# mathaiml5/NBody-simulation-parallel

Hardware: AMD Instinct MI355X
Metric: body-pair interactions/sec at N=2^20 (all-pairs force + kick/drift step) (higher is better)
Workload: dtype f32

## Files before the change

### nbody-simulation-parallel_amd/csrc/force_sym_kernel.hip

```cpp
#include "nbx_internal.h"
#include "sym_plan.h"

namespace nbx {
namespace {

typedef float f2 __attribute__((ext_vector_type(2)));

__device__ __forceinline__ float ror1(float v) {
    const int i = __builtin_bit_cast(int, v);
    return __builtin_bit_cast(float, __builtin_amdgcn_update_dpp(i, i, 0x13C, 0xF, 0xF, false));
}
__device__ __forceinline__ void ror1(f2& v) { v.x = ror1(v.x); v.y = ror1(v.y); }

enum { kRotDpp = 0, kRotLds = 1 };
template <int D> struct RotBuf { static constexpr unsigned kEntries = (D == 3) ? 128u : 72u; };

template <int D, int PAIRS>
__device__ __forceinline__ void sym_step(const f2 vxy, const f2 vzm, const f2 (&ix)[PAIRS], const f2 (&iy)[PAIRS],
                                         const f2 (&iz)[PAIRS], const f2 (&hm)[PAIRS], f2 (&ax)[PAIRS], f2 (&ay)[PAIRS],
                                         f2 (&az)[PAIRS], f2& vax, f2& vay, f2& vaz, const f2 bias) {
    f2 dx[PAIRS], dy[PAIRS], dz[PAIRS], r2[PAIRS], w[PAIRS], wh[PAIRS];
#pragma unroll
    for (int q = 0; q < PAIRS; ++q) dx[q] = __builtin_shufflevector(vxy, vxy, 0, 0) - ix[q];
#pragma unroll
    for (int q = 0; q < PAIRS; ++q) dy[q] = __builtin_shufflevector(vxy, vxy, 1, 1) - iy[q];
#pragma unroll
    for (int q = 0; q < PAIRS; ++q) dz[q] = (D == 3) ? __builtin_shufflevector(vzm, vzm, 0, 0) - iz[q] : f2{0.f, 0.f};
#pragma unroll
    for (int q = 0; q < PAIRS; ++q) r2[q] = __builtin_elementwise_fma(dx[q], dx[q], bias);
#pragma unroll
    for (int q = 0; q < PAIRS; ++q) r2[q] = __builtin_elementwise_fma(dy[q], dy[q], r2[q]);
    if (D == 3) {
#pragma unroll
        for (int q = 0; q < PAIRS; ++q) r2[q] = __builtin_elementwise_fma(dz[q], dz[q], r2[q]);
    }
#pragma unroll
    for (int q = 0; q < PAIRS; ++q) { w[q].x = __builtin_amdgcn_rcpf(r2[q].x); w[q].y = __builtin_amdgcn_rcpf(r2[q].y); }
#pragma unroll
    for (int q = 0; q < PAIRS; ++q) r2[q] = w[q] * w[q];
#pragma unroll
    for (int q = 0; q < PAIRS; ++q) w[q] = __builtin_shufflevector(vzm, vzm, 1, 1) * r2[q];
#pragma unroll
    for (int q = 0; q < PAIRS; ++q) wh[q] = hm[q] * r2[q];
#pragma unroll
    for (int q = 0; q < PAIRS; ++q) ax[q] = __builtin_elementwise_fma(w[q], dx[q], ax[q]);
#pragma unroll
    for (int q = 0; q < PAIRS; ++q) ay[q] = __builtin_elementwise_fma(w[q], dy[q], ay[q]);
    if (D == 3) {
#pragma unroll
        for (int q = 0; q < PAIRS; ++q) az[q] = __builtin_elementwise_fma(w[q], dz[q], az[q]);
    }
#pragma unroll
    for (int q = 0; q < PAIRS; ++q) {
        vax = __builtin_elementwise_fma(wh[q], dx[q], vax);
        vay = __builtin_elementwise_fma(wh[q], dy[q], vay);
        if (D == 3) vaz = __builtin_elementwise_fma(wh[q], dz[q], vaz);
    }
}

template <int D>
__device__ __forceinline__ void load_visitor(const float* __restrict__ tp, const float* __restrict__ mp, unsigned pad,
                                             unsigned v, f2& vxy, f2& vzm) {
    vxy = f2{tp[v], tp[(size_t)pad + v]};
    vzm = f2{(D == 3) ? tp[2 * (size_t)pad + v] : 0.0f, mp[v]};
}

__device__ __forceinline__ void store_hi_lo(float* __restrict__ hi_plane, float* __restrict__ lo_plane, size_t idx, double v) {
    const float hi = (float)v;
    hi_plane[idx] = hi;
    lo_plane[idx] = (float)(v - (double)hi);
}

template <int D, int QS, int ROT>
__global__ __launch_bounds__(256, 2) void accel_sym3l_kernel(KArgs a) {
    constexpr int PAIRS = 4;
    constexpr unsigned kSumBytes = (unsigned)PAIRS * D * 256u * sizeof(double2);
    constexpr unsigned kVisBytes = 4u * kSymChunkGroups * kSymGroup * sizeof(float4);
    constexpr unsigned kRotEntries = RotBuf<D>::kEntries;
    constexpr unsigned kRotBytes = (ROT == kRotLds) ? 4u * kRotEntries * sizeof(float4) : 0u;
    __shared__ __attribute__((aligned(16))) char smem[kSumBytes + kVisBytes + kRotBytes];
    double2* __restrict__ sums = reinterpret_cast<double2*>(smem);
    float4* __restrict__ vbuf = reinterpret_cast<float4*>(smem + kSumBytes);

    SymPlan P;
    if (!sym_make_plan(a.pad, &P) || P.B != gridDim.x || P.S != gridDim.y) return;
    const unsigned A = blockIdx.x, s = blockIdx.y;
    const unsigned tid = threadIdx.x, lane = tid & 63u, wave = tid >> 6;
    unsigned long long clk_r0 = 0, clk_t0 = 0;
    if (a.clk) {
        clk_r0 = __builtin_amdgcn_s_memrealtime();
        clk_t0 = __builtin_amdgcn_s_memtime();
        __builtin_amdgcn_s_waitcnt(0xC07F);
    }
    const size_t pad = a.pad;
    const float* __restrict__ tp = a.pos_all + (size_t)a.tgt_chunk * D * pad;
    const float* __restrict__ mp = a.mass_all + (size_t)a.tgt_chunk * pad;
    const f2 bias = f2{kTiny, kTiny};
    const size_t slot_stride = 2 * (size_t)D * pad;

    const unsigned delta = ((unsigned)__builtin_amdgcn_update_dpp((int)lane, (int)lane, 0x13C, 0xF, 0xF, false) - lane) & 63u;
    const unsigned rpos = ((0u - delta) * lane) & 63u;
    const unsigned vrot = kSumBytes + kVisBytes + ((ROT == kRotLds) ? wave * kRotEntries * (unsigned)sizeof(float4) : 0u);

    if (sym_clears_last_slot(P, A)) {
        float* __restrict__ hi = a.acc + (size_t)(P.S + P.K - 1u) * slot_stride;
        const unsigned len = kSymSuper / P.S;
        for (unsigned t = tid; t < len; t += 256u) {
            const size_t v = (size_t)A * kSymSuper + (size_t)s * len + t;
            if (v < pad) {
#pragma unroll
                for (int k = 0; k < 2 * D; ++k) hi[(size_t)k * pad + v] = 0.0f;
                if (QS) a.qsum[(size_t)(P.S + P.K - 1u) * pad + v] = 0.0f;
            }
        }
    }

    for (unsigned hp = 0; hp < kSymSuper / kSymHomePass; ++hp) {
        const unsigned h0 = A * kSymSuper + hp * kSymHomePass;
        if (h0 >= a.pad) break;
        const unsigned tgt0 = h0 + tid;
        f2 ix[PAIRS], iy[PAIRS], iz[PAIRS], hm[PAIRS], qq[QS ? PAIRS : 1];
#pragma unroll
        for (int q = 0; q < PAIRS; ++q) {
            const unsigned i0 = tgt0 + (2 * q) * 256u, i1 = i0 + 256u;
            ix[q] = f2{tp[i0], tp[i1]};
            iy[q] = f2{tp[pad + i0], tp[pad + i1]};
            iz[q] = (D == 3) ? f2{tp[2 * pad + i0], tp[2 * pad + i1]} : f2{0.f, 0.f};
            hm[q] = f2{mp[i0], mp[i1]};
            if (QS) qq[q] = f2{0.f, 0.f};
        }
#pragma unroll
        for (int c = 0; c < PAIRS * D; ++c) sums[c * 256 + tid] = double2{0.0, 0.0};

        SymWalk nw;
        nw.k = 0u; nw.c = ~0u;
        bool more = sym_next_chunk(P, A, s, &nw);
        f2 nxy = f2{0.f, 0.f}, nzm = f2{0.f, 0.f};
        if (more) load_visitor<D>(tp, mp, a.pad, nw.first + lane, nxy, nzm);
        while (more) {
            const SymWalk cw = nw;
            f2 ox[PAIRS], oy[PAIRS], oz[PAIRS];
#pragma unroll
            for (int q = 0; q < PAIRS; ++q) ox[q] = oy[q] = oz[q] = f2{0.f, 0.f};
#pragma unroll 1
            for (unsigned g = 0; g < cw.groups; ++g) {
                f2 vxy = nxy, vzm = nzm;
                if (g + 1u < cw.groups) {
                    load_visitor<D>(tp, mp, a.pad, cw.first + (g + 1u) * kSymGroup + lane, nxy, nzm);
                } else {
                    more = sym_next_chunk(P, A, s, &nw);
                    if (more) load_visitor<D>(tp, mp, a.pad, nw.first + lane, nxy, nzm);
                }
                float4* __restrict__ vslot = vbuf + (wave * kSymChunkGroups + g) * kSymGroup;
                vslot[lane] = make_float4(0.f, 0.f, 0.f, 0.f);
                unsigned roff = 0u;
                if (ROT == kRotLds) {
                    const float4 me = make_float4(vxy.x, vxy.y, vzm.x, vzm.y);
                    *reinterpret_cast<float4*>(smem + vrot + rpos * 16u) = me;
                    if (kRotEntries == 128u || rpos < kRotEntries - 64u) *reinterpret_cast<float4*>(smem + vrot + (rpos + 64u) * 16u) = me;
                    __builtin_amdgcn_fence(__ATOMIC_RELEASE, "wavefront");
                    __builtin_amdgcn_wave_barrier();
                    __builtin_amdgcn_fence(__ATOMIC_ACQUIRE, "wavefront");
                    roff = (kRotEntries == 128u) ? vrot + (rpos + 56u) * 16u : ((rpos + 56u) & 63u) * 16u;
                    asm volatile("" : "+v"(roff));
                }
                f2 ax[PAIRS], ay[PAIRS], az[PAIRS];
#pragma unroll
                for (int q = 0; q < PAIRS; ++q) ax[q] = ay[q] = az[q] = f2{0.f, 0.f};
#pragma unroll 1
                for (unsigned blk = 0; blk < 8u; ++blk) {
                    f2 vax = f2{0.f, 0.f}, vay = f2{0.f, 0.f}, vaz = f2{0.f, 0.f};
                    const char* rot = smem;
                    if (ROT == kRotLds) rot = smem + ((kRotEntries == 128u) ? roff : vrot + roff);
#pragma unroll
                    for (int j = 0; j < 8; ++j) {
                        if (ROT == kRotLds) {
                            asm volatile("" : "+v"(vzm));
                            const float4 nv = *reinterpret_cast<const float4*>(rot + (7 - j) * 16);
                            __builtin_amdgcn_sched_barrier(0);
                            sym_step<D, PAIRS>(vxy, vzm, ix, iy, iz, hm, ax, ay, az, vax, vay, vaz, bias);
                            vxy = f2{nv.x, nv.y}; vzm = f2{nv.z, nv.w};
                        } else {
                            sym_step<D, PAIRS>(vxy, vzm, ix, iy, iz, hm, ax, ay, az, vax, vay, vaz, bias);
                            ror1(vxy); ror1(vzm);
                        }
                        ror1(vax); ror1(vay);
                        if (D == 3) ror1(vaz);
                        __builtin_amdgcn_sched_barrier(0);
                    }
                    if (ROT == kRotLds) {
                        roff = (kRotEntries == 128u) ? roff - 128u : (roff - 128u) & 1023u;
                        asm volatile("" : "+v"(roff));
                    }
                    const unsigned vid = (lane + (blk + 1u) * 8u * delta) & 63u;
                    const float bx = vax.x + vax.y, by = vay.x + vay.y, bz = (D == 3) ? vaz.x + vaz.y : 0.0f;
                    float4 cur = vslot[vid];
                    cur.x += bx; cur.y += by; cur.z += bz;
                    if (QS) cur.w = __builtin_fmaf(bz, bz, __builtin_fmaf(by, by, __builtin_fmaf(bx, bx, cur.w)));
                    vslot[vid] = cur;
                }
#pragma unroll
                for (int q = 0; q < PAIRS; ++q) { ox[q] += ax[q]; oy[q] += ay[q]; if (D == 3) oz[q] += az[q]; }
                if (QS) {
#pragma unroll
                    for (int q = 0; q < PAIRS; ++q) {
                        qq[q] = __builtin_elementwise_fma(ax[q], ax[q], qq[q]);
                        qq[q] = __builtin_elementwise_fma(ay[q], ay[q], qq[q]);
                        if (D == 3) qq[q] = __builtin_elementwise_fma(az[q], az[q], qq[q]);
                    }
                }
            }
#pragma unroll
            for (int q = 0; q < PAIRS; ++q) {
                double2 v = sums[(q * D + 0) * 256 + tid];
                v.x += (double)ox[q].x; v.y += (double)ox[q].y;
                sums[(q * D + 0) * 256 + tid] = v;
                v = sums[(q * D + 1) * 256 + tid];
                v.x += (double)oy[q].x; v.y += (double)oy[q].y;
                sums[(q * D + 1) * 256 + tid] = v;
                if (D == 3) {
                    v = sums[(q * D + 2) * 256 + tid];
                    v.x += (double)oz[q].x; v.y += (double)oz[q].y;
                    sums[(q * D + 2) * 256 + tid] = v;
                }
            }
            if (!cw.two_sided) continue;
            __syncthreads();
            if (tid < cw.groups * kSymGroup) {
                const unsigned g = tid >> 6;
                const size_t v = (size_t)cw.first + tid;
                const float4 b0 = vbuf[(0u * kSymChunkGroups + g) * kSymGroup + lane], b1 = vbuf[(1u * kSymChunkGroups + g) * kSymGroup + lane];
                const float4 b2 = vbuf[(2u * kSymChunkGroups + g) * kSymGroup + lane], b3 = vbuf[(3u * kSymChunkGroups + g) * kSymGroup + lane];
                float* __restrict__ hi = a.acc + (size_t)(P.S + cw.k - 1u) * slot_stride;
                float* __restrict__ lo = hi + (size_t)D * pad;
                double rx = -((((double)b0.x + (double)b1.x) + (double)b2.x) + (double)b3.x);
                double ry = -((((double)b0.y + (double)b1.y) + (double)b2.y) + (double)b3.y);
                double rz = -((((double)b0.z + (double)b1.z) + (double)b2.z) + (double)b3.z);
                if (hp != 0u) {
                    rx += (double)hi[v] + (double)lo[v];
                    ry += (double)hi[pad + v] + (double)lo[pad + v];
                    if (D == 3) rz += (double)hi[2 * pad + v] + (double)lo[2 * pad + v];
                }
                store_hi_lo(hi, lo, v, rx);
                store_hi_lo(hi, lo, pad + v, ry);
                if (D == 3) store_hi_lo(hi, lo, 2 * pad + v, rz);
                if (QS) {
                    float* __restrict__ qo = a.qsum + (size_t)(P.S + cw.k - 1u) * pad + v;
                    const float qv = ((b0.w + b1.w) + b2.w) + b3.w;
                    *qo = (hp != 0u) ? *qo + qv : qv;
                }
            }
            __syncthreads();
        }

        float* __restrict__ hi = a.acc + (size_t)s * slot_stride;
        float* __restrict__ lo = hi + (size_t)D * pad;
        float* __restrict__ qout = QS ? a.qsum + (size_t)s * pad : nullptr;
#pragma unroll
        for (int q = 0; q < PAIRS; ++q) {
            const double2 vx = sums[(q * D + 0) * 256 + tid], vy = sums[(q * D + 1) * 256 + tid];
            const double2 vz = (D == 3) ? sums[(q * D + (D == 3 ? 2 : 0)) * 256 + tid] : double2{0.0, 0.0};
#pragma unroll
            for (int h = 0; h < 2; ++h) {
                const unsigned i = tgt0 + (2 * q + h) * 256u;
                if (!a.bad_flag[i]) {
                    store_hi_lo(hi, lo, i, h ? vx.y : vx.x);
                    store_hi_lo(hi, lo, pad + i, h ? vy.y : vy.x);
                    if (D == 3) store_hi_lo(hi, lo, 2 * pad + i, h ? vz.y : vz.x);
                    if (QS) qout[i] = h ? qq[q].y : qq[q].x;
                } else if (QS) {
                    qout[i] = __builtin_inff();
                }
            }
        }
    }
    if (a.clk) {
        const unsigned long long t1 = __builtin_amdgcn_s_memtime(), r1 = __builtin_amdgcn_s_memrealtime();
        if (tid == 0) {
            const size_t wg = (size_t)blockIdx.y * gridDim.x + blockIdx.x;
            a.clk[2 * wg] = t1 - clk_t0;
            a.clk[2 * wg + 1] = r1 - clk_r0;
        }
    }
}

}

namespace {
template <int ROT>
KernelVariant sym_variant(const char* name) {
    KernelVariant v = {};
    v.name = name;
    v.tpl = 8;
    v.k2 = accel_sym3l_kernel<2, 0, ROT>; v.k3 = accel_sym3l_kernel<3, 0, ROT>;
    v.qs2 = accel_sym3l_kernel<2, 1, ROT>; v.qs3 = accel_sym3l_kernel<3, 1, ROT>;
    v.fast = 1;
    v.planes = 2;
    v.sym = 1;
    v.stamps = 1;
    return v;
}
}
KernelVariant sym_kernel_variant() { return sym_variant<kRotLds>("sympk3l_t8_w3"); }
KernelVariant sym_dpp_kernel_variant() { return sym_variant<kRotDpp>("sympk3l_t8_w3_dpp"); }

}
```

Baseline: 6432 billion.

## Process two visitor groups per lane in 3D symmetric force kernel

For 3D, each lane now holds two visitor bodies (from adjacent groups) packed in f2 vectors rather than packing two home bodies per f2. Each step computes 8 home bodies against 2 visitors, so the visitor data rotated through LDS or DPP and the visitor reaction sums are amortized over twice as many interactions. The LDS rotation buffer becomes two 72-entry planes per wave instead of 128 entries. The trade-off is more registers for 8-way accumulators, a requirement of at least two groups per chunk, and duplicated code paths for 2D and 3D.

```diff
diff --git a/nbody-simulation-parallel_amd/csrc/force_sym_kernel.hip b/nbody-simulation-parallel_amd/csrc/force_sym_kernel.hip
--- a/nbody-simulation-parallel_amd/csrc/force_sym_kernel.hip
+++ b/nbody-simulation-parallel_amd/csrc/force_sym_kernel.hip
@@ -13,7 +13,13 @@
 __device__ __forceinline__ void ror1(f2& v) { v.x = ror1(v.x); v.y = ror1(v.y); }
 
 enum { kRotDpp = 0, kRotLds = 1 };
-template <int D> struct RotBuf { static constexpr unsigned kEntries = (D == 3) ? 128u : 72u; };
+template <int D> struct SymLanes { static constexpr int kVisitors = (D == 3) ? 2 : 1; };
+constexpr int kSymBlockSteps = 8;
+template <int D> struct RotBuf {
+    static constexpr unsigned kEntries = 72u;
+    static constexpr unsigned kPlanes = (unsigned)SymLanes<D>::kVisitors;
+    static constexpr unsigned kWaveBytes = kPlanes * kEntries * (unsigned)sizeof(float4);
+};
 
 template <int D, int PAIRS>
 __device__ __forceinline__ void sym_step(const f2 vxy, const f2 vzm, const f2 (&ix)[PAIRS], const f2 (&iy)[PAIRS],
@@ -65,6 +71,63 @@
     vzm = f2{(D == 3) ? tp[2 * (size_t)pad + v] : 0.0f, mp[v]};
 }
 
+template <int H> __device__ __forceinline__ f2 bcast(const f2 v) { return __builtin_shufflevector(v, v, H, H); }
+
+__device__ __forceinline__ void sym_step_pairs(const f2 vx, const f2 vy, const f2 vz, const f2 vm, const f2 (&ix)[4],
+                                               const f2 (&iy)[4], const f2 (&iz)[4], const f2 (&hm)[4], f2 (&ax)[8], f2 (&ay)[8],
+                                               f2 (&az)[8], f2& vax, f2& vay, f2& vaz, const f2 bias) {
+#pragma unroll
+    for (int b = 0; b < 2; ++b) {
+        f2 dx[4], dy[4], dz[4], r2[4], w[4], wh[4];
+#pragma unroll
+        for (int k = 0; k < 4; ++k) dx[k] = vx - ((k & 1) ? bcast<1>(ix[2 * b + k / 2]) : bcast<0>(ix[2 * b + k / 2]));
+#pragma unroll
+        for (int k = 0; k < 4; ++k) dy[k] = vy - ((k & 1) ? bcast<1>(iy[2 * b + k / 2]) : bcast<0>(iy[2 * b + k / 2]));
+#pragma unroll
+        for (int k = 0; k < 4; ++k) dz[k] = vz - ((k & 1) ? bcast<1>(iz[2 * b + k / 2]) : bcast<0>(iz[2 * b + k / 2]));
+#pragma unroll
+        for (int k = 0; k < 4; ++k) r2[k] = __builtin_elementwise_fma(dx[k], dx[k], bias);
+#pragma unroll
+        for (int k = 0; k < 4; ++k) r2[k] = __builtin_elementwise_fma(dy[k], dy[k], r2[k]);
+#pragma unroll
+        for (int k = 0; k < 4; ++k) r2[k] = __builtin_elementwise_fma(dz[k], dz[k], r2[k]);
+#pragma unroll
+        for (int k = 0; k < 4; ++k) { w[k].x = __builtin_amdgcn_rcpf(r2[k].x); w[k].y = __builtin_amdgcn_rcpf(r2[k].y); }
+#pragma unroll
+        for (int k = 0; k < 4; ++k) r2[k] = w[k] * w[k];
+#pragma unroll
+        for (int k = 0; k < 4; ++k) w[k] = vm * r2[k];
+#pragma unroll
+        for (int k = 0; k < 4; ++k) wh[k] = ((k & 1) ? bcast<1>(hm[2 * b + k / 2]) : bcast<0>(hm[2 * b + k / 2])) * r2[k];
+#pragma unroll
+        for (int k = 0; k < 4; ++k) ax[4 * b + k] = __builtin_elementwise_fma(w[k], dx[k], ax[4 * b + k]);
+#pragma unroll
+        for (int k = 0; k < 4; ++k) ay[4 * b + k] = __builtin_elementwise_fma(w[k], dy[k], ay[4 * b + k]);
+#pragma unroll
+        for (int k = 0; k < 4; ++k) az[4 * b + k] = __builtin_elementwise_fma(w[k], dz[k], az[4 * b + k]);
+#pragma unroll
+        for (int k = 0; k < 4; ++k) {
+            vax = __builtin_elementwise_fma(wh[k], dx[k], vax);
+            vay = __builtin_elementwise_fma(wh[k], dy[k], vay);
+            vaz = __builtin_elementwise_fma(wh[k], dz[k], vaz);
+        }
+        if (b == 0) __builtin_amdgcn_sched_barrier(0);
+    }
+}
+
+__device__ __forceinline__ void keep_packed(f2 (&ix)[4], f2 (&iy)[4], f2 (&iz)[4], f2 (&hm)[4]) {
+#pragma unroll
+    for (int q = 0; q < 4; ++q) asm volatile("" : "+v"(ix[q]), "+v"(iy[q]), "+v"(iz[q]), "+v"(hm[q]));
+}
+
+__device__ __forceinline__ void load_visitor_pair(const float* __restrict__ tp, const float* __restrict__ mp, unsigned pad,
+                                                  unsigned v, f2& vx, f2& vy, f2& vz, f2& vm) {
+    vx = f2{tp[v], tp[v + kSymGroup]};
+    vy = f2{tp[(size_t)pad + v], tp[(size_t)pad + v + kSymGroup]};
+    vz = f2{tp[2 * (size_t)pad + v], tp[2 * (size_t)pad + v + kSymGroup]};
+    vm = f2{mp[v], mp[v + kSymGroup]};
+}
+
 __device__ __forceinline__ void store_hi_lo(float* __restrict__ hi_plane, float* __restrict__ lo_plane, size_t idx, double v) {
     const float hi = (float)v;
     hi_plane[idx] = hi;
@@ -76,14 +139,16 @@
     constexpr int PAIRS = 4;
     constexpr unsigned kSumBytes = (unsigned)PAIRS * D * 256u * sizeof(double2);
     constexpr unsigned kVisBytes = 4u * kSymChunkGroups * kSymGroup * sizeof(float4);
+    constexpr int VPL = SymLanes<D>::kVisitors;
     constexpr unsigned kRotEntries = RotBuf<D>::kEntries;
-    constexpr unsigned kRotBytes = (ROT == kRotLds) ? 4u * kRotEntries * sizeof(float4) : 0u;
+    constexpr unsigned kRotBytes = (ROT == kRotLds) ? 4u * RotBuf<D>::kWaveBytes : 0u;
     __shared__ __attribute__((aligned(16))) char smem[kSumBytes + kVisBytes + kRotBytes];
     double2* __restrict__ sums = reinterpret_cast<double2*>(smem);
     float4* __restrict__ vbuf = reinterpret_cast<float4*>(smem + kSumBytes);
 
     SymPlan P;
     if (!sym_make_plan(a.pad, &P) || P.B != gridDim.x || P.S != gridDim.y) return;
+    if (VPL == 2 && P.G < 2u) return;
     const unsigned A = blockIdx.x, s = blockIdx.y;
     const unsigned tid = threadIdx.x, lane = tid & 63u, wave = tid >> 6;
     unsigned long long clk_r0 = 0, clk_t0 = 0;
@@ -100,7 +165,7 @@
 
     const unsigned delta = ((unsigned)__builtin_amdgcn_update_dpp((int)lane, (int)lane, 0x13C, 0xF, 0xF, false) - lane) & 63u;
     const unsigned rpos = ((0u - delta) * lane) & 63u;
-    const unsigned vrot = kSumBytes + kVisBytes + ((ROT == kRotLds) ? wave * kRotEntries * (unsigned)sizeof(float4) : 0u);
+    const unsigned vrot = kSumBytes + kVisBytes + ((ROT == kRotLds) ? wave * RotBuf<D>::kWaveBytes : 0u);
 
     if (sym_clears_last_slot(P, A)) {
         float* __restrict__ hi = a.acc + (size_t)(P.S + P.K - 1u) * slot_stride;
@@ -136,77 +201,175 @@
         nw.k = 0u; nw.c = ~0u;
         bool more = sym_next_chunk(P, A, s, &nw);
         f2 nxy = f2{0.f, 0.f}, nzm = f2{0.f, 0.f};
-        if (more) load_visitor<D>(tp, mp, a.pad, nw.first + lane, nxy, nzm);
+        f2 nvx = f2{0.f, 0.f}, nvy = f2{0.f, 0.f}, nvz = f2{0.f, 0.f}, nvm = f2{0.f, 0.f};
+        if (more) {
+            if constexpr (VPL == 2) load_visitor_pair(tp, mp, a.pad, nw.first + lane, nvx, nvy, nvz, nvm);
+            else load_visitor<D>(tp, mp, a.pad, nw.first + lane, nxy, nzm);
+        }
         while (more) {
             const SymWalk cw = nw;
             f2 ox[PAIRS], oy[PAIRS], oz[PAIRS];
 #pragma unroll
             for (int q = 0; q < PAIRS; ++q) ox[q] = oy[q] = oz[q] = f2{0.f, 0.f};
+            if constexpr (VPL == 2) {
 #pragma unroll 1
-            for (unsigned g = 0; g < cw.groups; ++g) {
-                f2 vxy = nxy, vzm = nzm;
-                if (g + 1u < cw.groups) {
-                    load_visitor<D>(tp, mp, a.pad, cw.first + (g + 1u) * kSymGroup + lane, nxy, nzm);
-                } else {
-                    more = sym_next_chunk(P, A, s, &nw);
-                    if (more) load_visitor<D>(tp, mp, a.pad, nw.first + lane, nxy, nzm);
-                }
-                float4* __restrict__ vslot = vbuf + (wave * kSymChunkGroups + g) * kSymGroup;
-                vslot[lane] = make_float4(0.f, 0.f, 0.f, 0.f);
-                unsigned roff = 0u;
-                if (ROT == kRotLds) {
-                    const float4 me = make_float4(vxy.x, vxy.y, vzm.x, vzm.y);
-                    *reinterpret_cast<float4*>(smem + vrot + rpos * 16u) = me;
-                    if (kRotEntries == 128u || rpos < kRotEntries - 64u) *reinterpret_cast<float4*>(smem + vrot + (rpos + 64u) * 16u) = me;
-                    __builtin_amdgcn_fence(__ATOMIC_RELEASE, "wavefront");
-                    __builtin_amdgcn_wave_barrier();
-                    __builtin_amdgcn_fence(__ATOMIC_ACQUIRE, "wavefront");
-                    roff = (kRotEntries == 128u) ? vrot + (rpos + 56u) * 16u : ((rpos + 56u) & 63u) * 16u;
-                    asm volatile("" : "+v"(roff));
-                }
-                f2 ax[PAIRS], ay[PAIRS], az[PAIRS];
-#pragma unroll
-                for (int q = 0; q < PAIRS; ++q) ax[q] = ay[q] = az[q] = f2{0.f, 0.f};
+                for (unsigned g = 0; g < cw.groups; g += 2u) {
+                    f2 vx = nvx, vy = nvy, vz = nvz, vm = nvm;
+                    if (g + 2u < cw.groups) {
+                        load_visitor_pair(tp, mp, a.pad, cw.first + (g + 2u) * kSymGroup + lane, nvx, nvy, nvz, nvm);
+                    } else {
+                        more = sym_next_chunk(P, A, s, &nw);
+                        if (more) load_visitor_pair(tp, mp, a.pad, nw.first + lane, nvx, nvy, nvz, nvm);
+                    }
+                    float4* __restrict__ vslot = vbuf + (wave * kSymChunkGroups + g) * kSymGroup;
+                    vslot[lane] = make_float4(0.f, 0.f, 0.f, 0.f);
+                    vslot[kSymGroup + lane] = make_float4(0.f, 0.f, 0.f, 0.f);
+                    constexpr unsigned kPlane = kRotEntries * (unsigned)sizeof(float4);
+                    constexpr unsigned kBlockBytes = (unsigned)kSymBlockSteps * (unsigned)sizeof(float4);
+                    unsigned roff = 0u;
+                    if (ROT == kRotLds) {
+                        const float4 lo4 = make_float4(vx.x, vx.y, vy.x, vy.y), hi4 = make_float4(vz.x, vz.y, vm.x, vm.y);
+                        *reinterpret_cast<float4*>(smem + vrot + rpos * 16u) = lo4;
+                        *reinterpret_cast<float4*>(smem + vrot + kPlane + rpos * 16u) = hi4;
+                        if (rpos < kRotEntries - 64u) {
+                            *reinterpret_cast<float4*>(smem + vrot + (rpos + 64u) * 16u) = lo4;
+                            *reinterpret_cast<float4*>(smem + vrot + kPlane + (rpos + 64u) * 16u) = hi4;
+                        }
+                        __builtin_amdgcn_fence(__ATOMIC_RELEASE, "wavefront");
+                        __builtin_amdgcn_wave_barrier();
+                        __builtin_amdgcn_fence(__ATOMIC_ACQUIRE, "wavefront");
+                        roff = ((rpos + 64u - (unsigned)kSymBlockSteps) & 63u) * 16u;
+                        asm volatile("" : "+v"(roff));
+                    }
+                    f2 ax[2 * PAIRS], ay[2 * PAIRS], az[2 * PAIRS];
+#pragma unroll
+                    for (int k = 0; k < 2 * PAIRS; ++k) ax[k] = ay[k] = az[k] = f2{0.f, 0.f};
 #pragma unroll 1
-                for (unsigned blk = 0; blk < 8u; ++blk) {
-                    f2 vax = f2{0.f, 0.f}, vay = f2{0.f, 0.f}, vaz = f2{0.f, 0.f};
-                    const char* rot = smem;
-                    if (ROT == kRotLds) rot = smem + ((kRotEntries == 128u) ? roff : vrot + roff);
-#pragma unroll
-                    for (int j = 0; j < 8; ++j) {
+                    for (unsigned blk = 0; blk < kSymGroup / (unsigned)kSymBlockSteps; ++blk) {
+                        f2 vax = f2{0.f, 0.f}, vay = f2{0.f, 0.f}, vaz = f2{0.f, 0.f};
+                        const char* rot = smem;
+                        if (ROT == kRotLds) rot = smem + (vrot + roff);
+#pragma unroll
+                        for (int j = 0; j < kSymBlockSteps; ++j) {
+                            if (ROT == kRotLds) {
+                                asm volatile("" : "+v"(vx), "+v"(vy), "+v"(vz), "+v"(vm));
+                                const float4 n0 = *reinterpret_cast<const float4*>(rot + (kSymBlockSteps - 1 - j) * 16);
+                                const float4 n1 = *reinterpret_cast<const float4*>(rot + kPlane + (kSymBlockSteps - 1 - j) * 16);
+                                __builtin_amdgcn_sched_barrier(0);
+                                keep_packed(ix, iy, iz, hm);
+                                sym_step_pairs(vx, vy, vz, vm, ix, iy, iz, hm, ax, ay, az, vax, vay, vaz, bias);
+                                vx = f2{n0.x, n0.y}; vy = f2{n0.z, n0.w}; vz = f2{n1.x, n1.y}; vm = f2{n1.z, n1.w};
+                            } else {
+                                keep_packed(ix, iy, iz, hm);
+                                sym_step_pairs(vx, vy, vz, vm, ix, iy, iz, hm, ax, ay, az, vax, vay, vaz, bias);
+                                ror1(vx); ror1(vy); ror1(vz); ror1(vm);
+                            }
+                            ror1(vax); ror1(vay); ror1(vaz);
+                            __builtin_amdgcn_sched_barrier(0);
+                        }
                         if (ROT == kRotLds) {
-                            asm volatile("" : "+v"(vzm));
-                            const float4 nv = *reinterpret_cast<const float4*>(rot + (7 - j) * 16);
+                            roff = (roff - kBlockBytes) & 1023u;
+                            asm volatile("" : "+v"(roff));
+                        }
+                        const unsigned vid = (lane + (blk + 1u) * (unsigned)kSymBlockSteps * delta) & 63u;
+                        float4 c0 = vslot[vid], c1 = vslot[kSymGroup + vid];
+                        c0.x += vax.x; c0.y += vay.x; c0.z += vaz.x;
+                        c1.x += vax.y; c1.y += vay.y; c1.z += vaz.y;
+                        if (QS) {
+                            c0.w = __builtin_fmaf(vaz.x, vaz.x, __builtin_fmaf(vay.x, vay.x, __builtin_fmaf(vax.x, vax.x, c0.w)));
+                            c1.w = __builtin_fmaf(vaz.y, vaz.y, __builtin_fmaf(vay.y, vay.y, __builtin_fmaf(vax.y, vax.y, c1.w)));
+                        }
+                        vslot[vid] = c0;
+                        vslot[kSymGroup + vid] = c1;
+                    }
+#pragma unroll
+                    for (int q = 0; q < PAIRS; ++q) {
+                        ox[q].x += ax[2 * q].x; oy[q].x += ay[2 * q].x; oz[q].x += az[2 * q].x;
+                        ox[q].y += ax[2 * q + 1].x; oy[q].y += ay[2 * q + 1].x; oz[q].y += az[2 * q + 1].x;
+                        ox[q].x += ax[2 * q].y; oy[q].x += ay[2 * q].y; oz[q].x += az[2 * q].y;
+                        ox[q].y += ax[2 * q + 1].y; oy[q].y += ay[2 * q + 1].y; oz[q].y += az[2 * q + 1].y;
+                    }
+                    if (QS) {
+#pragma unroll
+                        for (int q = 0; q < PAIRS; ++q) {
+                            const f2 x0 = f2{ax[2 * q].x, ax[2 * q + 1].x}, y0 = f2{ay[2 * q].x, ay[2 * q + 1].x}, z0 = f2{az[2 * q].x, az[2 * q + 1].x};
+                            const f2 x1 = f2{ax[2 * q].y, ax[2 * q + 1].y}, y1 = f2{ay[2 * q].y, ay[2 * q + 1].y}, z1 = f2{az[2 * q].y, az[2 * q + 1].y};
+                            qq[q] = __builtin_elementwise_fma(x0, x0, qq[q]);
+                            qq[q] = __builtin_elementwise_fma(y0, y0, qq[q]);
+                            qq[q] = __builtin_elementwise_fma(z0, z0, qq[q]);
+                            qq[q] = __builtin_elementwise_fma(x1, x1, qq[q]);
+                            qq[q] = __builtin_elementwise_fma(y1, y1, qq[q]);
+                            qq[q] = __builtin_elementwise_fma(z1, z1, qq[q]);
+                        }
+                    }
+                }
+            } else {
+#pragma unroll 1
+                for (unsigned g = 0; g < cw.groups; ++g) {
+                    f2 vxy = nxy, vzm = nzm;
+                    if (g + 1u < cw.groups) {
+                        load_visitor<D>(tp, mp, a.pad, cw.first + (g + 1u) * kSymGroup + lane, nxy, nzm);
+                    } else {
+                        more = sym_next_chunk(P, A, s, &nw);
+                        if (more) load_visitor<D>(tp, mp, a.pad, nw.first + lane, nxy, nzm);
+                    }
+                    float4* __restrict__ vslot = vbuf + (wave * kSymChunkGroups + g) * kSymGroup;
+                    vslot[lane] = make_float4(0.f, 0.f, 0.f, 0.f);
+                    unsigned roff = 0u;
+                    if (ROT == kRotLds) {
+                        const float4 me = make_float4(vxy.x, vxy.y, vzm.x, vzm.y);
+                        *reinterpret_cast<float4*>(smem + vrot + rpos * 16u) = me;
+                        if (rpos < kRotEntries - 64u) *reinterpret_cast<float4*>(smem + vrot + (rpos + 64u) * 16u) = me;
+                        __builtin_amdgcn_fence(__ATOMIC_RELEASE, "wavefront");
+                        __builtin_amdgcn_wave_barrier();
+                        __builtin_amdgcn_fence(__ATOMIC_ACQUIRE, "wavefront");
+                        roff = ((rpos + 56u) & 63u) * 16u;
+                        asm volatile("" : "+v"(roff));
+                    }
+                    f2 ax[PAIRS], ay[PAIRS], az[PAIRS];
+#pragma unroll
+                    for (int q = 0; q < PAIRS; ++q) ax[q] = ay[q] = az[q] = f2{0.f, 0.f};
+#pragma unroll 1
+                    for (unsigned blk = 0; blk < 8u; ++blk) {
+                        f2 vax = f2{0.f, 0.f}, vay = f2{0.f, 0.f}, vaz = f2{0.f, 0.f};
+                        const char* rot = smem;
+                        if (ROT == kRotLds) rot = smem + (vrot + roff);
+#pragma unroll
+                        for (int j = 0; j < 8; ++j) {
+                            if (ROT == kRotLds) {
+                                asm volatile("" : "+v"(vzm));
+                                const float4 nv = *reinterpret_cast<const float4*>(rot + (7 - j) * 16);
+                                __builtin_amdgcn_sched_barrier(0);
+                                sym_step<D, PAIRS>(vxy, vzm, ix, iy, iz, hm, ax, ay, az, vax, vay, vaz, bias);
+                                vxy = f2{nv.x, nv.y}; vzm = f2{nv.z, nv.w};
+                            } else {
+                                sym_step<D, PAIRS>(vxy, vzm, ix, iy, iz, hm, ax, ay, az, vax, vay, vaz, bias);
+                                ror1(vxy); ror1(vzm);
+                            }
+                            ror1(vax); ror1(vay);
+                            if (D == 3) ror1(vaz);
                             __builtin_amdgcn_sched_barrier(0);
-                            sym_step<D, PAIRS>(vxy, vzm, ix, iy, iz, hm, ax, ay, az, vax, vay, vaz, bias);
-                            vxy = f2{nv.x, nv.y}; vzm = f2{nv.z, nv.w};
-                        } else {
-                            sym_step<D, PAIRS>(vxy, vzm, ix, iy, iz, hm, ax, ay, az, vax, vay, vaz, bias);
-                            ror1(vxy); ror1(vzm);
-                        }
-                        ror1(vax); ror1(vay);
-                        if (D == 3) ror1(vaz);
-                        __builtin_amdgcn_sched_barrier(0);
-                    }
-                    if (ROT == kRotLds) {
-                        roff = (kRotEntries == 128u) ? roff - 128u : (roff - 128u) & 1023u;
-                        asm volatile("" : "+v"(roff));
-                    }
-                    const unsigned vid = (lane + (blk + 1u) * 8u * delta) & 63u;
-                    const float bx = vax.x + vax.y, by = vay.x + vay.y, bz = (D == 3) ? vaz.x + vaz.y : 0.0f;
-                    float4 cur = vslot[vid];
-                    cur.x += bx; cur.y += by; cur.z += bz;
-                    if (QS) cur.w = __builtin_fmaf(bz, bz, __builtin_fmaf(by, by, __builtin_fmaf(bx, bx, cur.w)));
-                    vslot[vid] = cur;
-                }
-#pragma unroll
-                for (int q = 0; q < PAIRS; ++q) { ox[q] += ax[q]; oy[q] += ay[q]; if (D == 3) oz[q] += az[q]; }
-                if (QS) {
-#pragma unroll
-                    for (int q = 0; q < PAIRS; ++q) {
-                        qq[q] = __builtin_elementwise_fma(ax[q], ax[q], qq[q]);
-                        qq[q] = __builtin_elementwise_fma(ay[q], ay[q], qq[q]);
-                        if (D == 3) qq[q] = __builtin_elementwise_fma(az[q], az[q], qq[q]);
+                        }
+                        if (ROT == kRotLds) {
+                            roff = (roff - 128u) & 1023u;
+                            asm volatile("" : "+v"(roff));
+                        }
+                        const unsigned vid = (lane + (blk + 1u) * 8u * delta) & 63u;
+                        const float bx = vax.x + vax.y, by = vay.x + vay.y, bz = (D == 3) ? vaz.x + vaz.y : 0.0f;
+                        float4 cur = vslot[vid];
+                        cur.x += bx; cur.y += by; cur.z += bz;
+                        if (QS) cur.w = __builtin_fmaf(bz, bz, __builtin_fmaf(by, by, __builtin_fmaf(bx, bx, cur.w)));
+                        vslot[vid] = cur;
+                    }
+#pragma unroll
+                    for (int q = 0; q < PAIRS; ++q) { ox[q] += ax[q]; oy[q] += ay[q]; if (D == 3) oz[q] += az[q]; }
+                    if (QS) {
+#pragma unroll
+                        for (int q = 0; q < PAIRS; ++q) {
+                            qq[q] = __builtin_elementwise_fma(ax[q], ax[q], qq[q]);
+                            qq[q] = __builtin_elementwise_fma(ay[q], ay[q], qq[q]);
+                            if (D == 3) qq[q] = __builtin_elementwise_fma(az[q], az[q], qq[q]);
+                        }
                     }
                 }
             }
```

New measurement: 6558 billion, median of 6. 2.0% higher.
